# daysun/grid_ndt

Measured on AMD Instinct MI355X. Metric: NDT grid-build throughput (bin + mean/cov + eigen + labels + ordering), higher is better.
Workload: dtype f64

## Files before the change

grid_ndt_amd/_lib.py:

```python
import ctypes as C
import os
import subprocess

_CSRC = os.path.join(os.path.dirname(os.path.abspath(__file__)), "csrc")
_ROOT = os.path.dirname(os.path.dirname(os.path.abspath(__file__)))
LIB_PATH = os.path.join(_CSRC, "libgndt.so")
SOURCES = ["gndt_api_core.hip", "gndt_api_table.hip", "gndt_api_build.hip", "gndt_api_dist.hip", "gndt_api_cost.hip", "gndt_api_query.hip",
           "gndt_api_crop.hip", "gndt_api_raster.hip", "gndt_api_clear.hip", "gndt_api_io.hip", "gndt_codec.cpp", "gndt_io.cpp"]
HEADERS = ["gndt_handle.hpp", "gndt_kernels.hpp", "gndt_table.hpp", "gndt_cost.hpp", "gndt_query.hpp", "gndt_ray.hpp", "gndt_crop.hpp", "gndt_pack.hpp", "gndt_partition.hpp", "gndt_bucket3.hpp", "gndt_blocked.hpp", "gndt_tile.hpp", "gndt_exchange.hpp", "gndt_math.hpp", os.path.join(_ROOT, "include", "gndt.h")]

GNDT_OK = 0
ERR_NAMES = {0: "OK", 1: "INVALID", 2: "NO_DEVICE", 3: "HIP", 4: "KEY_RANGE", 5: "CAPACITY", 6: "NOMEM", 7: "PEER"}


class GndtError(RuntimeError):
    def __init__(self, code, msg):
        super().__init__(f"gndt error {code} ({ERR_NAMES.get(code, '?')}): {msg}")
        self.code = code


class Params(C.Structure):
    _fields_ = [("grid_len", C.c_float), ("z_len", C.c_float), ("slope_interval", C.c_float),
                ("demand", C.c_int32), ("min_points", C.c_int32), ("device_id", C.c_int32),
                ("strategy", C.c_int32), ("max_points_hint", C.c_uint64), ("max_nodes_hint", C.c_uint64)]
# ... 146 lines not shown
    L.gndt_build.argtypes = [H, vp, sz, sz]
    L.gndt_build_device.argtypes = [H, vp, sz, sz, vp]
    L.gndt_update.argtypes = [H, vp, sz, sz]
    L.gndt_update_device.argtypes = [H, vp, sz, sz, vp]
    L.gndt_remove.argtypes = [H, vp, sz, sz]
    L.gndt_remove_device.argtypes = [H, vp, sz, sz, vp]
    L.gndt_reset.argtypes = [H, vp]
    L.gndt_accumulate_device.argtypes = [H, vp, sz, sz, u64, vp]
    L.gndt_finalize_device.argtypes = [H, vp]
    L.gndt_sync.argtypes = [H, C.POINTER(u64), C.POINTER(u64), C.POINTER(u64)]
    L.gndt_export_device.argtypes = [H, C.POINTER(Cells)]
    L.gndt_export.argtypes = [H, C.POINTER(Cells)]
    L.gndt_export_host.argtypes = [H, C.POINTER(Cells)]
    L.gndt_reserve.argtypes = [H, u64, u64]
    L.gndt_set_deferred_emit.argtypes = [H, C.c_int]
    L.gndt_set_deferred_emit.restype = C.c_int
    L.gndt_reserve.restype = C.c_int
    L.gndt_export_host.restype = C.c_int
    L.gndt_stats_export_device.argtypes = [H, C.POINTER(Stats), vp]
    L.gndt_stats_merge_device.argtypes = [H, C.POINTER(Stats), vp]
    L.gndt_shard_stats_device.argtypes = [H, vp, C.c_size_t, C.c_size_t, u64, C.POINTER(Stats), vp]
    L.gndt_finalize_stats_device.argtypes = [H, C.POINTER(Stats), u64, vp]
    L.gndt_get_origin.argtypes = [H, C.POINTER(C.c_float)]
    L.gndt_pcd_read.argtypes = [C.c_char_p, C.POINTER(Pcd), C.c_char_p]
    L.gndt_pcd_free.argtypes = [C.POINTER(Pcd)]
    L.gndt_pcd_free.restype = None
    L.gndt_pack_points_device.argtypes = [H, vp, C.c_size_t, C.POINTER(PointLayout), vp, C.POINTER(u64), vp]
    L.gndt_build_cloud.argtypes = [H, vp, C.c_size_t, C.POINTER(PointLayout)]
    L.gndt_compute_cost.argtypes = [H, C.POINTER(C.c_float), C.POINTER(Robot), vp]
    L.gndt_cost_export_device.argtypes = [H, C.POINTER(vp), C.POINTER(vp), C.POINTER(CostStats)]
    L.gndt_cost_export.argtypes = [H, vp, vp, C.POINTER(CostStats)]
    L.gndt_query_device.argtypes = [H, vp, sz, sz, C.c_int32, vp, vp, vp, vp]
    L.gndt_query.argtypes = [H, vp, sz, sz, C.c_int32, vp, vp, vp]
    L.gndt_crop_device.argtypes = [H, C.POINTER(CropBox), C.c_int32, vp]
    L.gndt_crop.argtypes = [H, C.POINTER(CropBox), C.c_int32]
    L.gndt_crop_box_from_world.argtypes = [C.POINTER(C.c_float), C.c_float, C.POINTER(C.c_float), C.POINTER(C.c_float), C.POINTER(CropBox)]
    L.gndt_raster_shape.argtypes = [C.POINTER(CropBox), C.POINTER(C.c_uint32), C.POINTER(C.c_uint32)]
    L.gndt_raster_device.argtypes = [H, C.POINTER(CropBox), C.c_int32, C.c_float, C.POINTER(RasterLayers), vp]
    L.gndt_raster.argtypes = [H, C.POINTER(CropBox), C.c_int32, C.c_float, C.POINTER(RasterLayers)]
    L.gndt_clear_rays_device.argtypes = [H, C.POINTER(C.c_float), vp, sz, sz, C.POINTER(ClearParams), vp, C.POINTER(ClearStats), vp]
    L.gndt_clear_rays.argtypes = [H, C.POINTER(C.c_float), vp, sz, sz, C.POINTER(ClearParams), vp, C.POINTER(ClearStats)]
    L.gndt_trans_morton_xyz.argtypes = [C.POINTER(C.c_float), C.c_float, C.c_float, C.POINTER(C.c_float), C.c_char_p,
                                        C.POINTER(C.c_int32), C.POINTER(C.c_int32), C.POINTER(C.c_int32), C.c_char_p]
    L.gndt_count_morton.argtypes = [C.c_int32, C.c_int32, C.c_char_p]
    L.gndt_morton_to_xy.argtypes = [C.c_int32, C.POINTER(C.c_int32), C.POINTER(C.c_int32)]
    L.gndt_pack_key.argtypes = [C.c_int32, C.c_int32, C.c_int32]
    L.gndt_pack_key.restype = u64
    L.gndt_unpack_key.argtypes = [u64, C.POINTER(C.c_int32), C.POINTER(C.c_int32), C.POINTER(C.c_int32)]
    L.gndt_unpack_key.restype = None
    L.gndt_set_profiling.argtypes = [H, C.c_int]
    L.gndt_get_phase_times.argtypes = [H, C.POINTER(C.c_double)]
    L.gndt_debug_bucket_phases.argtypes = [H, C.POINTER(C.c_double), C.POINTER(C.c_uint32)]
    L.gndt_debug_bucket_phases.restype = C.c_int
    L.gndt_debug_retry_count.argtypes = [H, C.POINTER(u64)]
    L.gndt_debug_retry_count.restype = C.c_int
    L.gndt_debug_enable_stamps.argtypes = [C.c_int]
    L.gndt_debug_enable_stamps.restype = C.c_int
    L.gndt_warmup.argtypes = [C.c_void_p, C.c_uint64]
    L.gndt_warmup.restype = C.c_int
    L.gndt_debug_set_option.argtypes = [C.c_int, C.c_double]
    L.gndt_debug_set_option.restype = C.c_int
    L.gndt_debug_set_fp_bits.argtypes = [C.c_int]
    L.gndt_debug_set_fp_bits.restype = C.c_int
    L.gndt_debug_fp_clashes.argtypes = [H, C.POINTER(u64)]
    L.gndt_debug_fp_clashes.restype = C.c_int
    L.gndt_debug_second_pass_buckets.argtypes = [H, C.POINTER(u64)]
    L.gndt_debug_second_pass_buckets.restype = C.c_int
    L.gndt_debug_fail_next_alloc.argtypes = [H, C.c_int]
    L.gndt_debug_fail_next_alloc.restype = C.c_int
    L.gndt_comm_unique_id.argtypes = [C.c_char_p]
    L.gndt_comm_create.argtypes = [C.c_char_p, C.c_int32, C.c_int32, C.c_int32, C.POINTER(vp)]
    L.gndt_comm_destroy.argtypes = [vp]
    L.gndt_comm_create_threads.argtypes = [C.c_int32, C.c_int32, C.POINTER(vp)]
    L.gndt_comm_create_threads.restype = C.c_int
    L.gndt_comm_destroy.restype = None
    L.gndt_comm_last_error.restype = C.c_char_p
    L.gndt_comm_selftest.argtypes = [H, vp, C.POINTER(CommSelftest), vp]
    L.gndt_comm_selftest.restype = C.c_int
    L.gndt_build_global_device.argtypes = [H, vp, vp, C.c_size_t, C.c_size_t, u64, u64, C.POINTER(ExchangeTimes), vp]
    L.gndt_owner_of_columns.argtypes = [vp, vp, C.c_size_t, C.c_uint32, vp]
    L.gndt_owner_of_columns.restype = C.c_int
    L.gndt_owner_sample_device.argtypes = [H, vp, C.c_size_t, C.c_size_t, C.POINTER(vp), C.POINTER(u64), vp]
    L.gndt_owner_map_device.argtypes = [H, vp, C.c_uint32, vp]
    L.gndt_owner_sample_device.restype = L.gndt_owner_map_device.restype = C.c_int
    L.gndt_owner_split_device.argtypes = [H, vp, C.c_size_t, C.c_size_t, u64, u64, C.c_uint32, C.POINTER(vp), C.POINTER(u64), C.POINTER(u64), vp]
    L.gndt_build_records_device.argtypes = [H, vp, C.c_size_t, u64, vp]
    L.gndt_build_records2_device.argtypes = [H, vp, C.c_size_t, vp, C.c_size_t, u64, vp]
    L.gndt_build_records2_device.restype = C.c_int
    L.gndt_owned_columns_device.argtypes = [H, C.POINTER(vp), C.POINTER(u64), vp]
    L.gndt_owned_global_rows_device.argtypes = [H, vp, u64, u64, C.POINTER(vp), C.POINTER(u64), C.POINTER(u64), vp]
    L.gndt_build_owned_device.argtypes = [H, vp, vp, C.c_size_t, C.c_size_t, u64, u64, C.POINTER(vp), C.POINTER(OwnedInfo), vp]
    L.gndt_gather_owned_map_device.argtypes = [H, vp, C.c_int32, vp]
    L.gndt_owned_pack_rows_device.argtypes = [H, C.POINTER(vp), C.POINTER(u64), vp]
    L.gndt_adopt_rows_device.argtypes = [H, vp, u64, u64, u64, u64, vp]
    for name in ("gndt_gather_owned_map_device", "gndt_owned_pack_rows_device", "gndt_adopt_rows_device"):
        getattr(L, name).restype = C.c_int
    for name in ("gndt_comm_unique_id", "gndt_comm_create", "gndt_build_global_device", "gndt_owner_split_device",
                 "gndt_build_records_device", "gndt_owned_columns_device", "gndt_owned_global_rows_device", "gndt_build_owned_device"):
        getattr(L, name).restype = C.c_int
    L.gndt_locality_sample.argtypes = [H, vp, C.c_size_t, C.c_size_t, C.c_uint32, C.POINTER(C.c_double), vp]
    L.gndt_locality_sample.restype = C.c_int
    L.gndt_last_strategy.argtypes = [H]
    L.gndt_last_strategy.restype = C.c_int
    L.gndt_device_info.argtypes = [C.c_int32, C.c_char_p, C.POINTER(C.c_int32), C.POINTER(u64)]
    for name in ("gndt_create", "gndt_set_origin", "gndt_build", "gndt_build_device", "gndt_update", "gndt_update_device",
                 "gndt_remove", "gndt_remove_device",
# ... 11 lines not shown
```

grid_ndt_amd/csrc/gndt_api_build.hip:

```cpp
#include <atomic>

#include "gndt_handle.hpp"
#include "gndt_bucket3.hpp"
#include "gndt_blocked.hpp"
using namespace gndt;
using namespace gndt_host;

namespace gndt_host {

int launch_order_and_emit(gndt_handle* h, uint64_t words, int m0, hipStream_t s, bool grouped, bool counters_to_host, bool tab_end, uint32_t advance,
                          bool partial) {
    auto& q = h->part;
    const bool dest_scans = grouped && !partial && !tab_end && words <= kDestScanMax && tuning().dest_scans;
    if (dest_scans) {
    } else if (words <= kScanSmallMax) {
        hipLaunchKernelGGL(k_scan_small, dim3(1), dim3(1024), 0, s, (const uint32_t*)q.word_weight, (uint32_t)words, q.word_base);
    } else {
        const uint32_t nbw = (uint32_t)((words + kScanChunk - 1) / kScanChunk);
        hipLaunchKernelGGL(k_scan_reduce<false>, dim3(nbw), dim3(kScanThreads), 0, s, q.word_weight, (const uint32_t*)nullptr,
                           (uint32_t)words, q.bsum_words);
        hipLaunchKernelGGL(k_scan_apply<false>, dim3(nbw), dim3(kScanThreads), 0, s, q.word_weight, (const uint32_t*)nullptr,
                           (uint32_t)words, q.bsum_words, q.word_base);
    }
    HIP_TRY(h, hipGetLastError());
// ... 478 lines not shown
    h->results_valid = false;
    h->map_in_table = false;
    h->stream_pos = index_range ? index_range : n;
    h->last_stream = s;
    return GNDT_OK;
}

int partition_recheck_after_replay(gndt_handle* h) {
    auto& P = h->pending;
    auto& q = h->part;
    if (P.active || !P.done_serial || P.done_serial != h->result_serial || P.stats_only || P.records || h->map_in_table || !q.h_pc ||
        (!h->results_valid && !P.replay_failed))
        return GNDT_OK;
    if (!(q.h_pc->part_overflow | q.h_pc->lds_overflow | q.h_pc->stage_overflow)) {
        if (P.replay_failed) { P.replay_failed = false; h->results_valid = true; }
        return GNDT_OK;
    }
    h->results_valid = false;
    P.replay_failed = true;
    h->err = "a build replayed from a hipGraph ran out of room (LDS tables " + std::to_string(q.h_pc->lds_overflow) + ", partition regions " +
             std::to_string(q.h_pc->part_overflow) + ", staging rows " + std::to_string(q.h_pc->stage_overflow) +
             "): the capture is sized for the cloud it was recorded on — build this cloud eagerly (gndt_build_device + gndt_sync), then capture again";
    return GNDT_ERR_CAPACITY;
}

static void blocked_decide(gndt_handle* h, const gndt_handle::Pending& P) {
    auto& q = h->part;
    const uint64_t n = P.n + P.n2;
    if (!tuning().blocked || P.stats_only || P.records || P.captured || !P.two_level || P.blocked || h->ever_captured) return;
    if (h->P.strategy != GNDT_STRATEGY_AUTO && h->P.strategy != GNDT_STRATEGY_PARTITION && h->P.strategy != GNDT_STRATEGY_PARTITION_TWO_LEVEL) return;
    if (q.blk_state != 0 && n <= q.blk_n + q.blk_n / 4 && n + n / 4 >= q.blk_n) return;
    q.blk_state = -1; q.blk_n = n;
    if (!(q.pair_ratio >= 0.0 && q.pair_ratio <= 0.02)) return;
    const uint64_t nodes = h->h_cnt->num_nodes;
    if (nodes < 1024 || nodes > h->out_cap) return;
    hipStream_t s = P.s;
    if (!q.d_extent) {
        if (hipMalloc(&q.d_extent, 8 * sizeof(uint32_t)) != hipSuccess) { (void)hipGetLastError(); return; }
        if (hipHostMalloc(&q.h_extent, 8 * sizeof(uint32_t)) != hipSuccess) { (void)hipGetLastError(); return; }
    }
    for (int k = 0; k < 8; ++k) q.h_extent[k] = k < 3 ? 0xFFFFFFFFu : 0u;
    if (hipMemcpyAsync(q.d_extent, q.h_extent, 8 * sizeof(uint32_t), hipMemcpyHostToDevice, s) != hipSuccess) { (void)hipGetLastError(); return; }
    hipLaunchKernelGGL(k_key_extent, dim3(64), dim3(1024), 0, s, (const int32_t*)h->out.sx, (const int32_t*)h->out.sy, (const int32_t*)h->out.sz,
                       (const uint32_t*)h->out.count, (uint32_t)nodes, q.d_extent);
    if (hipMemcpyAsync(q.h_extent, q.d_extent, 8 * sizeof(uint32_t), hipMemcpyDeviceToHost, s) != hipSuccess || hipStreamSynchronize(s) != hipSuccess) {
        (void)hipGetLastError();
        return;
    }
    const int64_t bias = 1ll << 30;
    const int64_t x0 = (int64_t)q.h_extent[0] - bias, y0 = (int64_t)q.h_extent[1] - bias, z0 = (int64_t)q.h_extent[2] - bias;
    const int64_t X = (int64_t)q.h_extent[3] - bias - x0 + 1, Y = (int64_t)q.h_extent[4] - bias - y0 + 1, Z = (int64_t)q.h_extent[5] - bias - z0 + 1;
    const uint64_t biggest = q.h_extent[6];
    if (X <= 0 || Y <= 0 || Z <= 0 || Z > 32) return;
    int shz = 0;
    while ((1 << shz) < Z) ++shz;
    for (; shz <= 5; ++shz) {
        const int shx = (9 - shz + 1) / 2, shy = 9 - shz - shx;
        const uint64_t nx = (uint64_t)((X + (1ll << shx) - 1) >> shx), ny = (uint64_t)((Y + (1ll << shy) - 1) >> shy);
        const uint64_t B = nx * ny;
        if (B < 64 || B > (uint64_t)kMaxFan * kMaxFan) continue;
        const uint64_t per_block = n / B;
        if (per_block > 5000) continue;
        if (per_block < 1500) break;
        if (biggest * 4 > per_block) break;
        if (nodes * 8 < B * 512) break;
        const int64_t zpad = ((1ll << shz) - Z) / 2;
        q.blk_map = BlockMap{1, (int)(x0 - (1ll << shx)), (int)(y0 - (1ll << shy)), (int)(z0 - zpad), shx, shy, shz, (int)nx + 2, (int)ny + 2};
        q.blk_buckets = (uint32_t)((nx + 2) * (ny + 2));
        if (q.blk_buckets > (uint64_t)kMaxFan * kMaxFan) { q.blk_map.on = 0; continue; }
        q.blk_state = 1;
        if (tuning().verbose)
            fprintf(stderr, "[gndt] blocked buckets for clouds of ~%llu points: box %lld x %lld x %lld, blocks of %d x %d columns x %d levels, %llu buckets of ~%llu points\n",
                    (unsigned long long)n, (long long)X, (long long)Y, (long long)Z, 1 << shx, 1 << shy, 1 << shz, (unsigned long long)B, (unsigned long long)per_block);
        return;
    }
}

int partition_resolve(gndt_handle* h) {
    auto& P = h->pending;
    if (!P.active) return GNDT_OK;
    auto& q = h->part;
    const int env_slots = tuning().bucket_slots;
    int rc = GNDT_OK;
    for (;;) {
        if (hipStreamSynchronize(P.s) != hipSuccess) { P.active = false; h->err = "hipStreamSynchronize failed"; return GNDT_ERR_HIP; }
        bool again = false;
        if (P.two_level && P.mean1 > 0) {
            q.fill1_ratio = q.h_pc->max_fill1 / P.mean1;
            if (tuning().verbose)
                fprintf(stderr, "[gndt] two-level partition: fullest level-1 region %.2fx the mean, overflow %u\n",
                        q.h_pc->max_fill1 / P.mean1, q.h_pc->part_overflow);
        }
        if (tuning().verbose && (q.h_pc->part_overflow | q.h_pc->lds_overflow | q.h_pc->stage_overflow))
            fprintf(stderr, "[gndt] build of %zu points, attempt %d (%d-slot tables, %llu nodes expected): region overflow %u, table overflow %u, "
                            "staging overflow %u -> re-run\n", P.n, P.attempt, P.bslots, (unsigned long long)P.nodes_est, q.h_pc->part_overflow,
                    q.h_pc->lds_overflow, q.h_pc->stage_overflow);
        if (P.blocked && (q.h_pc->blk_miss | q.h_pc->part_overflow)) {
            q.blk_state = -1;
            P.no_block = true;
            --P.attempt;
            again = true;
        } else if (q.h_pc->part_overflow) {
            if (P.one_level) q.one_level_ok = false;
            else ++q.two_level_failures;
            --P.attempt;
            again = true;
        } else if (q.h_pc->lds_overflow) {
            const bool without_retry = P.bslots == 512 && !P.retry_pass && tuning().retry_pass != 0 && !env_slots;
            q.retry_pass = true;
            const uint64_t b1024 = buckets_for(P.n + P.n2, P.nodes_est, 1024, P.load_pct ? P.load_pct : q.load_pct);
            if (without_retry) {
                --P.attempt;
            } else if (P.bslots == 512 && !env_slots && P.n + P.n2 <= (1u << 20) && b1024 < 384 && (P.load_pct ? P.load_pct : q.load_pct) > 35) {
                P.load_pct = 35;
                --P.attempt;
            } else if (P.attempt >= 1 || env_slots) {
                const bool few = q.h_pc->lds_overflow * 64u <= q.last_buckets;
                P.nodes_est = few ? P.nodes_est + (P.nodes_est * 2) / 5 : P.nodes_est * 2;
            }
            again = true;
        } else if (q.h_pc->stage_overflow) {
            const uint64_t true_nodes = h->h_cnt->num_nodes;
            const uint64_t want = true_nodes + true_nodes / 8 + 1024;
            if (want > P.stage_want) --P.attempt;
            P.stage_want = want;
            P.rows_floor = want;
// ... 141 lines not shown
        HIP_TRY(h, hipMalloc(&q.bucket_base, ((size_t)Bexact + 1) * 4));
        q.bucket_cap = (uint32_t)Bexact;
    }
    if ((rc = reserve_table(h, std::max<uint64_t>(max_nodes, std::max<uint64_t>(1024, n / 4)), h->own_stream))) return rc;
    HIP_TRY(h, hipStreamSynchronize(h->own_stream));
    if ((rc = ensure_stage(h, std::max<uint64_t>(1024, h->cap / 2 + 1)))) return rc;
    if ((rc = ensure_raw(h, q.stage_cap))) return rc;
    if ((rc = ensure_out(h, q.stage_cap))) return rc;
    return GNDT_OK;
}

int gndt_debug_retry_count(gndt_handle* h, uint64_t* retries) {
    if (!h || !retries) return GNDT_ERR_INVALID;
    *retries = h->part.retries_total;
    return GNDT_OK;
}

int gndt_debug_second_pass_buckets(gndt_handle* h, uint64_t* buckets) {
    if (!h || !buckets) return GNDT_ERR_INVALID;
    *buckets = h->part.retry_seen;
    return GNDT_OK;
}

int gndt_debug_enable_stamps(int on) { tuning_force_stamps(on != 0); return GNDT_OK; }
int gndt_debug_set_option(int option, double value) { return tuning_set_option(option, value); }

int gndt_debug_set_fp_bits(int bits) { tuning_force_fp_bits(bits); return GNDT_OK; }

int gndt_debug_fp_clashes(gndt_handle* h, uint64_t* buckets) {
    if (!h || !buckets) return GNDT_ERR_INVALID;
    *buckets = h->part.h_pc ? h->part.h_pc->fp_clashes : 0;
    return GNDT_OK;
}

int gndt_debug_bucket_phases(gndt_handle* h, double cycles_out[10], uint32_t* buckets_out) {
    if (!h || !cycles_out) return GNDT_ERR_INVALID;
    auto& q = h->part;
    if (!q.dbg || !q.last_buckets) { h->err = "no stamps: call gndt_debug_enable_stamps(1) before a PARTITION build"; return GNDT_ERR_INVALID; }
    HIP_TRY(h, hipSetDevice(h->device));
    HIP_TRY(h, hipStreamSynchronize(h->last_stream));
    std::vector<unsigned long long> t((size_t)q.last_buckets * 16);
    HIP_TRY(h, hipMemcpy(t.data(), q.dbg, t.size() * sizeof(unsigned long long), hipMemcpyDeviceToHost));
    for (int k = 0; k < 10; ++k) cycles_out[k] = 0.0;
    for (uint32_t b = 0; b < q.last_buckets; ++b) {
        const unsigned long long* s = &t[(size_t)b * 16];
        for (int k = 0; k < 6; ++k) if (s[k + 1] > s[k]) cycles_out[k] += (double)(s[k + 1] - s[k]);
        for (int k = 0; k < 4; ++k) cycles_out[6 + k] += (double)s[8 + k];
    }
    for (int k = 0; k < 10; ++k) cycles_out[k] /= q.last_buckets;
    if (buckets_out) *buckets_out = q.last_buckets;
    return GNDT_OK;
}

}

namespace {
__global__ void k_warm_fill(float* __restrict__ xyz, uint32_t n, uint32_t stride_floats, float gl, float zl) {
    for (uint32_t i = blockIdx.x * blockDim.x + threadIdx.x; i < n; i += gridDim.x * blockDim.x) {
        uint32_t a = i * 0x9E3779B1u + 0x7F4A7C15u; a ^= a >> 15; a *= 0x85EBCA77u; a ^= a >> 13;
        uint32_t b = a * 0xC2B2AE3Du + 0x165667B1u; b ^= b >> 16;
        uint32_t c = b * 0x27D4EB2Fu + 0x9E3779B1u; c ^= c >> 15;
        float* p = xyz + (size_t)i * stride_floats;
        p[0] = ((float)(a >> 8) * (1.0f / 16777216.0f) - 0.5f) * 100.0f * gl;
        p[1] = ((float)(b >> 8) * (1.0f / 16777216.0f) - 0.5f) * 100.0f * gl;
        p[2] = ((float)(c >> 8) * (1.0f / 16777216.0f) - 0.5f) * 4.0f * zl;
        if (stride_floats == 4) p[3] = 0.f;
    }
}
std::atomic<uint64_t> g_warm_points[64];
}

int gndt_warmup(gndt_handle* h, uint64_t expected_points) {
    if (!h) return GNDT_ERR_INVALID;
    HIP_TRY(h, hipSetDevice(h->device));
    {
        hipStreamCaptureStatus cap = hipStreamCaptureStatusNone;
        (void)hipStreamIsCapturing(h->own_stream, &cap);
        if (cap != hipStreamCaptureStatusNone) { h->err = "gndt_warmup: not under stream capture"; return GNDT_ERR_INVALID; }
    }
    uint64_t n = expected_points ? expected_points : (h->P.max_points_hint ? h->P.max_points_hint : 200000);
    const uint64_t reserve_points = expected_points ? expected_points : h->P.max_points_hint;
    n = std::min<uint64_t>(std::max<uint64_t>(n, 1u << 16), 4u << 20);
    const bool known_device = h->device >= 0 && h->device < 64;
    int rc = GNDT_OK;
    const uint64_t seen = known_device ? g_warm_points[h->device].load(std::memory_order_acquire) : 0;
    const bool loaded = seen && n <= seen + seen / 4 && n + n / 4 >= seen;
    if (!loaded) {
        hipStream_t s = h->own_stream;
        float* cloud = nullptr;
        HIP_TRY(h, hipMalloc(&cloud, (size_t)n * 16));
        auto run = [&](int strategy, uint32_t stride_floats, bool update, bool flood) -> int {
            gndt_params tp = h->P;
            tp.strategy = strategy; tp.max_points_hint = 0; tp.max_nodes_hint = 0;
            gndt_handle* t = nullptr;
            int r = create_handle(&tp, &t, s);
            if (r) { h->err = std::string("gndt_warmup: ") + gndt_last_error(nullptr); return r; }
            const float origin[3] = {0.f, 0.f, 0.f};
            hipLaunchKernelGGL(k_warm_fill, dim3(512), dim3(256), 0, s, cloud, (uint32_t)n, stride_floats, tp.grid_len, tp.z_len);
            r = gndt_set_origin(t, origin);
            for (int k = 0; k < 2 && !r; ++k) {
                r = gndt_build_device(t, cloud, (size_t)n, stride_floats * 4u, nullptr);
                if (!r) r = gndt_sync(t, nullptr, nullptr, nullptr);
            }
            if (!r && update) {
                r = gndt_update_device(t, cloud, (size_t)std::min<uint64_t>(n, 1u << 17), stride_floats * 4u, nullptr);
                if (!r) r = gndt_sync(t, nullptr, nullptr, nullptr);
// ... 26 lines not shown
```

grid_ndt_amd/csrc/gndt_blocked.hpp:

```cpp
#pragma once
#include <hip/hip_runtime.h>
#include <stdint.h>

#include "gndt_bucket3.hpp"

namespace gndt {

constexpr uint32_t kBlkChunk = 2048;
constexpr int kBlkPer = (int)kBlkChunk / 512;
constexpr uint32_t kBlkNone = 0xFFFFFFFFu;
struct BlockedLds {
    float4 image[kBlkChunk];
    uint32_t hist[2][512];
    uint32_t wpre[2][8];
    uint2 fz[512];
    uint32_t cpre[512];
    uint32_t wave_tot[8];
    uint32_t n_nodes, n_cols, n_slopes, stage_base, err_range, miss;
};

template <int T>
__global__ void __launch_bounds__(T) __attribute__((amdgpu_waves_per_eu(6, 6))) k_bucket_blocked(const float4* __restrict__ recs, BucketRanges ranges, uint32_t num_buckets, GridParams P,
                                                      RawNode* __restrict__ stage, uint32_t stage_cap,
                                                      uint32_t* __restrict__ ord_cf, uint32_t* __restrict__ ord_idx, ColumnOrder O,
                                                      Counters* __restrict__ cnt, PartCounters* __restrict__ pc,
                                                      unsigned long long* __restrict__ dbg) {
    static_assert(T == 512, "one table slot per thread");
    __shared__ BlockedLds L;
    const int tid = threadIdx.x;
    const BlockMap K = P.blk;
    const int sh_xy = K.shx + K.shy;
    const uint32_t col_mask = (1u << sh_xy) - 1u, n_levels = 1u << K.shz;
    if (blockIdx.x == 0 && tid == 0) { const uint32_t e = pc->l1_err; if (e) atomicAdd(&cnt->err_key_range, e); }
    for (uint32_t bucket = blockIdx.x; bucket < num_buckets; bucket += gridDim.x) {
#define GNDT_STAMPB(k) do { if (dbg && tid == 0) dbg[(size_t)bucket * 16 + (k)] = __builtin_amdgcn_s_memtime(); } while (0)
        uint32_t lo, hi;
        bucket_range(ranges, bucket, lo, hi);
        GNDT_STAMPB(0);
        const int bx0 = K.x0 + (int)((bucket / (uint32_t)K.ny) << K.shx), by0 = K.y0 + (int)((bucket % (uint32_t)K.ny) << K.shy);
        uint32_t s = (uint32_t)tid;
        asm volatile("" : "+v"(s));
        const uint32_t zero = s - (uint32_t)tid;
        float f_len = P.grid_len, f_zlen = P.z_len, f_ox = P.ox, f_oy = P.oy, f_oz = P.oz;
        asm volatile("" : "+s"(f_len), "+s"(f_zlen), "+s"(f_ox), "+s"(f_oy), "+s"(f_oz));
        const double hx = 0.5 * (double)f_len, hz = 0.5 * (double)f_zlen;
        const double ox = (double)f_ox, oy = (double)f_oy, oz = (double)f_oz;
        L.hist[0][s] = zero; L.hist[1][s] = zero;
        if (s < 16) L.wpre[s >> 3][s & 7] = zero;
        if (s == 0) { L.n_nodes = zero; L.n_cols = zero; L.n_slopes = zero; L.stage_base = zero; L.err_range = zero; L.miss = zero; }
        lds_barrier();
        GNDT_STAMPB(1);
        const uint32_t col = s & col_mask, lz = s >> sh_xy;
        const int cxi = bx0 + (int)(col & ((1u << K.shx) - 1u)), cyi = by0 + (int)(col >> K.shx), czi = K.z0 + (int)lz;
        const int nsx = cxi >= 0 ? cxi + 1 : cxi, nsy = cyi >= 0 ? cyi + 1 : cyi, nsz = czi >= 0 ? czi + 1 : czi;
        const double ctx = fma((double)(float)(nsx > 0 ? 2 * nsx - 1 : 2 * nsx + 1), hx, ox),
                     cty = fma((double)(float)(nsy > 0 ? 2 * nsy - 1 : 2 * nsy + 1), hx, oy),
                     ctz = fma((double)(float)(nsz > 0 ? 2 * nsz - 1 : 2 * nsz + 1), hz, oz);
        const uint32_t n_rec = hi - lo, n_chunks = (n_rec + kBlkChunk - 1u) / kBlkChunk;
        uint32_t my_n = 0, my_first = 0xFFFFFFFFu;
        double sums[9];
#pragma unroll
        for (int j = 0; j < 9; ++j) sums[j] = 0.0;
        float4 rec[kBlkPer];
#pragma unroll
        for (int j = 0; j < kBlkPer; ++j) rec[j] = make_float4(0.f, 0.f, 0.f, 0.f);
        if (lo < hi) {
#pragma unroll
            for (int j = 0; j < kBlkPer; ++j) rec[j] = recs[min(lo + (uint32_t)(j * T + tid), hi - 1u)];
        }
        for (uint32_t ch = 0; ch < n_chunks; ++ch) {
            const uint32_t par = ch & 1u, c0 = lo + ch * kBlkChunk;
            uint32_t slot_rank[kBlkPer];
#pragma unroll
            for (int j = 0; j < kBlkPer; ++j) {
                bool use = c0 + (uint32_t)(j * T + tid) < hi;
                bool und = false;
                float fx = axis_ceil_try(rec[j].x, P.ox, P.inv_grid, und);
                float fy = axis_ceil_try(rec[j].y, P.oy, P.inv_grid, und);
                float fz = axis_ceil_try(rec[j].z, P.oz, P.inv_z, und);
                if (und) {
                    fx = ceilf(fabsf(rec[j].x - P.ox) / P.grid_len);
                    fy = ceilf(fabsf(rec[j].y - P.oy) / P.grid_len);
                    fz = ceilf(fabsf(rec[j].z - P.oz) / P.z_len);
                }
                bool ok = true;
                int sx, sy, sz;
                double v0, v1, v2;
                axis_index_offset(rec[j].x, P.ox, fx, (float)kMaxXY, hx, ox, ok, sx, v0);
                axis_index_offset(rec[j].y, P.oy, fy, (float)kMaxXY, hx, oy, ok, sy, v1);
                axis_index_offset(rec[j].z, P.oz, fz, (float)kMaxZ, hz, oz, ok, sz, v2);
                (void)v0; (void)v1; (void)v2;
                if (use && !ok) { atomicAdd(&L.err_range, 1u); use = false; }
                const uint32_t lx = (uint32_t)(contiguous_index(sx) - bx0), ly = (uint32_t)(contiguous_index(sy) - by0),
                               lz2 = (uint32_t)(contiguous_index(sz) - K.z0);
                if (use && ((lx >> K.shx) | (ly >> K.shy) | (lz2 >> K.shz)) != 0u) { L.miss = 1u; use = false; }
                const uint32_t rs = (lz2 << sh_xy) | (ly << K.shx) | lx;
                slot_rank[j] = use ? (rs << 16) | atomicAdd(&L.hist[par][rs], 1u) : kBlkNone;
            }
            lds_barrier();
            {
                const uint32_t c = L.hist[par][s];
                uint32_t incl = c;
                const int lane = tid & 63, wv = tid >> 6;
                for (int off = 1; off < 64; off <<= 1) { const uint32_t t = (uint32_t)__shfl_up((int)incl, off, 64); if (lane >= off) incl += t; }
                const uint32_t wtot = (uint32_t)__shfl((int)incl, 63, 64);
                L.hist[par][s] = incl - c;
                if (lane > wv && lane < T / 64 && wtot) atomicAdd(&L.wpre[par][lane], wtot);
                L.hist[par ^ 1u][s] = 0u;
                if (tid < T / 64) L.wpre[par ^ 1u][tid] = 0u;
                lds_barrier();
#pragma unroll
                for (int j = 0; j < kBlkPer; ++j) {
                    const uint32_t sr = slot_rank[j];
                    if (sr != kBlkNone) L.image[L.hist[par][sr >> 16] + L.wpre[par][sr >> 22] + (sr & 0xFFFFu)] = rec[j];
                }
                const uint32_t b0 = incl - c + L.wpre[par][wv];
                if (ch + 1u < n_chunks) {
#pragma unroll
                    for (int j = 0; j < kBlkPer; ++j) rec[j] = recs[min(c0 + kBlkChunk + (uint32_t)(j * T + tid), hi - 1u)];
                }
                lds_barrier();
#pragma unroll 1
                for (uint32_t i = b0; i < b0 + c; ++i) {
                    const float4 r = L.image[i];
                    const double v0 = (double)r.x - ctx, v1 = (double)r.y - cty, v2 = (double)r.z - ctz;
                    const uint32_t iw = __float_as_uint(r.w);
                    uint32_t cn = 1u, cf = iw;
                    double w0 = v0, w1 = v1, w2 = v2;
                    if (__any((iw & kWeight64Flag) != 0u)) {
                        cn = record_weight(iw); cf = record_index(iw);
                        const double wf = (double)cn;
                        w0 = wf * v0; w1 = wf * v1; w2 = wf * v2;
                    }
                    my_n += cn; my_first = min(my_first, cf);
                    sums[0] += w0; sums[1] += w1; sums[2] += w2;
                    sums[3] += w0 * v0; sums[4] += w0 * v1; sums[5] += w0 * v2;
                    sums[6] += w1 * v1; sums[7] += w1 * v2; sums[8] += w2 * v2;
                }
            }
        }
        const bool live = my_n != 0u;
        {
            const uint32_t w = (uint32_t)__popcll(__ballot(live));
            if ((tid & 63) == 0 && w) atomicAdd(&L.n_nodes, w);
        }
        lds_barrier();
        GNDT_STAMPB(2);
        if (L.miss) {
            if (tid == 0) atomicAdd(&pc->blk_miss, 1u);
            lds_barrier();
            continue;
        }
        const uint32_t M = L.n_nodes;
        uint32_t stage_base_reg = 0;
        if (tid == T - 1 && M) stage_base_reg = atomicAdd(&cnt->num_nodes, M);
        if (tid == 0 && L.err_range) atomicAdd(&cnt->err_key_range, L.err_range);
        const float cz = (live && my_n >= (uint32_t)P.min_points) ? node_mean_z(my_n, sums[2], axis_centre(nsz, P.oz, P.z_len)) : 0.f;
        L.fz[s] = make_uint2(my_first, __float_as_uint(cz));
        lds_barrier();
        uint32_t icol = 0, ncol = 0, cfirst = 0xFFFFFFFFu;
        bool up = false, down = false;
        if (live || s <= col_mask) {
            for (uint32_t k0 = 0; k0 < n_levels; k0 += 4) {
                uint2 tt[4];
#pragma unroll
                for (int j = 0; j < 4; ++j) tt[j] = L.fz[min(((k0 + (uint32_t)j) << sh_xy) | col, 511u)];
#pragma unroll
                for (int j = 0; j < 4; ++j) {
                    const uint32_t k = k0 + (uint32_t)j, tf = tt[j].x;
                    if (k >= n_levels || tf == 0xFFFFFFFFu) continue;
                    ++ncol;
                    cfirst = min(cfirst, tf);
                    if (k == lz) continue;
                    icol += (tf < my_first) ? 1u : 0u;
                    if (k == lz + 1u || k + 1u == lz) {
                        const float oz2 = (tf < my_first) ? __uint_as_float(tt[j].y) : 0.f;
                        const bool far = fabsf(oz2 - cz) > P.slope_interval;
                        if (k == lz + 1u) up = far; else down = far;
                    }
                }
            }
        }
        {
            const uint32_t my_col_nodes = s <= col_mask ? ncol : 0u;
            uint32_t incl = my_col_nodes;
            const int lane = tid & 63;
            for (int off = 1; off < 64; off <<= 1) { const uint32_t t = (uint32_t)__shfl_up((int)incl, off, 64); if (lane >= off) incl += t; }
            if (s <= col_mask) L.cpre[s] = incl - my_col_nodes;
            if (lane == 63) L.wave_tot[tid >> 6] = incl;
            if (s <= col_mask && my_col_nodes) atomicAdd(&L.n_cols, 1u);
            if (tid == T - 1) L.stage_base = stage_base_reg;
            lds_barrier();
        }
        GNDT_STAMPB(3);
        const uint32_t sbase = L.stage_base;
        if (sbase + M > stage_cap) {
            if (tid == 0 && M) atomicAdd(&pc->stage_overflow, M);
            lds_barrier();
            continue;
        }
        uint32_t my_slopes = 0;
        if (live) {
            uint32_t fl = (my_n >= (uint32_t)P.min_points) ? 1u : 0u;
            if (fl) {
                bool slope = true;
                if (P.demand == 0) slope = !up; else down = false;
                if (slope) { fl |= 2u; if (down) fl |= 4u; ++my_slopes; }
            }
            RawNode row;
            row.key = pack_key(nsx, nsy, nsz); row.count = my_n; row.first = my_first;
#pragma unroll
            for (int j = 0; j < 9; ++j) row.sum[j] = sums[j];
            row.info = fl | (icol << 3);
            row.ncol = ncol;
            uint32_t cbase = L.cpre[col];
            for (uint32_t w = 0; w < (col >> 6); ++w) cbase += L.wave_tot[w];
            const uint32_t dst = sbase + cbase + icol;
            stage[dst] = row;
            ord_cf[dst] = cfirst;
            ord_idx[dst] = icol ? icol : (kOrdHeadFlag | ncol);
            if (icol == 0) note_column(O, cfirst, ncol);
        }
        if (my_slopes) atomicAdd(&L.n_slopes, my_slopes);
        lds_barrier();
        if (tid == 0) {
            if (L.n_cols | L.n_slopes) atomicAdd(&pc->cols_slopes, ((unsigned long long)L.n_slopes << 32) | (unsigned long long)L.n_cols);
        }
        GNDT_STAMPB(4);
        lds_barrier();
#undef GNDT_STAMPB
    }
}

static __global__ void __launch_bounds__(1024) k_key_extent(const int32_t* __restrict__ sx, const int32_t* __restrict__ sy, const int32_t* __restrict__ sz,
                                                            const uint32_t* __restrict__ count, uint32_t n, uint32_t* __restrict__ out) {
    __shared__ uint32_t red[7];
    if (threadIdx.x < 3) red[threadIdx.x] = 0xFFFFFFFFu;
    else if (threadIdx.x < 7) red[threadIdx.x] = 0u;
    __syncthreads();
    uint32_t mn[3] = {0xFFFFFFFFu, 0xFFFFFFFFu, 0xFFFFFFFFu}, mx[3] = {0u, 0u, 0u}, big = 0u;
    for (uint32_t i = blockIdx.x * blockDim.x + threadIdx.x; i < n; i += gridDim.x * blockDim.x) {
        const uint32_t c[3] = {(uint32_t)(contiguous_index(sx[i]) + (1 << 30)), (uint32_t)(contiguous_index(sy[i]) + (1 << 30)),
                               (uint32_t)(contiguous_index(sz[i]) + (1 << 30))};
#pragma unroll
        for (int k = 0; k < 3; ++k) { mn[k] = min(mn[k], c[k]); mx[k] = max(mx[k], c[k]); }
        big = max(big, count[i]);
    }
#pragma unroll
    for (int k = 0; k < 3; ++k) {
        for (int off = 32; off > 0; off >>= 1) {
            mn[k] = min(mn[k], (uint32_t)__shfl_down((int)mn[k], off, 64));
            mx[k] = max(mx[k], (uint32_t)__shfl_down((int)mx[k], off, 64));
        }
    }
    for (int off = 32; off > 0; off >>= 1) big = max(big, (uint32_t)__shfl_down((int)big, off, 64));
    if ((threadIdx.x & 63) == 0) {
#pragma unroll
        for (int k = 0; k < 3; ++k) { atomicMin(&red[k], mn[k]); atomicMax(&red[3 + k], mx[k]); }
        atomicMax(&red[6], big);
    }
    __syncthreads();
    if (threadIdx.x < 3) atomicMin(&out[threadIdx.x], red[threadIdx.x]);
    else if (threadIdx.x < 7) atomicMax(&out[threadIdx.x], red[threadIdx.x]);
}

}
```

grid_ndt_amd/csrc/gndt_kernels.hpp:

```cpp
#pragma once
#include <hip/hip_runtime.h>
#include <stdint.h>

#include "gndt_math.hpp"

namespace gndt {

struct NodeAcc {
    double s[9];
    uint32_t count;
    uint32_t first;
};
static_assert(sizeof(NodeAcc) == 80, "NodeAcc layout");

struct SlotAux {
    float mean_z;
    uint32_t flags;
};

struct Counters {
    uint32_t num_nodes;
    uint32_t num_columns;
    uint32_t num_slopes;
    uint32_t err_key_range;
    uint32_t err_table_full;
    uint32_t stream_pos;
    uint32_t prev_nodes;
    uint32_t epoch;
    uint32_t n_touched;
    uint32_t n_tcols;
    uint32_t n_work;
    uint32_t n_dead;
    uint32_t err_remove;
    uint32_t first_word;
    uint32_t ticket;
    uint32_t table_gen;
    uint32_t table_unclean;
    uint32_t part_owned;
};

struct BlockMap {
    int on;
    int x0, y0, z0;
    int shx, shy, shz;
    int nx, ny;
};
struct GridParams {
    float ox, oy, oz;
    float grid_len, z_len, slope_interval;
    int demand, min_points;
    float inv_grid, inv_z;
    BlockMap blk;
};

struct OutView {
    int32_t *sx, *sy, *sz;
    uint32_t *count, *first_idx;
    float *mean, *cov, *rough, *normal;
    uint32_t* flags;
};

constexpr int kBlock = 256;

__device__ __forceinline__ uint32_t find_or_insert(uint64_t* __restrict__ keys, uint32_t cap_mask, uint64_t key,
                                                   bool& inserted) {
    inserted = false;
    uint32_t slot = (uint32_t)mix64(key) & cap_mask;
    for (uint32_t probe = 0; probe <= cap_mask; ++probe) {
        uint64_t k = keys[slot];
        if (k == key) return slot;
        if (k == kEmptyKey) {
            unsigned long long old = atomicCAS((unsigned long long*)&keys[slot], (unsigned long long)kEmptyKey,
                                               (unsigned long long)key);
            if (old == kEmptyKey) { inserted = true; return slot; }
            if (old == key) return slot;
        }
        slot = (slot + 1) & cap_mask;
    }
    return cap_mask + 1;
}

__device__ __forceinline__ void append_new_nodes(bool inserted, uint32_t slot, uint32_t* __restrict__ node_slot,
                                                 uint32_t* __restrict__ index_of_slot, Counters* __restrict__ cnt) {
    const unsigned long long m = __ballot(inserted);
    if (m == 0ull) return;
    const int lane = threadIdx.x & 63;
    const int leader = (int)__builtin_ctzll(m);
    uint32_t base = 0;
    if (lane == leader) base = atomicAdd(&cnt->num_nodes, (uint32_t)__popcll(m));
    base = (uint32_t)__shfl((int)base, leader, 64);
    if (inserted) {
        const uint32_t idx = base + (uint32_t)__popcll(m & ((1ull << lane) - 1ull));
        node_slot[idx] = slot;
        index_of_slot[slot] = idx;
    }
}

// ... 351 lines not shown
```

grid_ndt_amd/map2d.py:

```python
import ctypes as C
import os

import numpy as np

from . import _lib
from ._lib import Cells, ClearParams, ClearStats, CropBox, CostStats, ExchangeTimes, GndtError, OwnedInfo, Params, Pcd, PointLayout, RasterLayers, Robot, Stats

DEMANDS = {"slope": 0, "true": 1}
FLAG_HAS_STATS, FLAG_SLOPE, FLAG_DOWN = 1, 2, 4


_HIP_STREAM_LEGACY = 1


def _stream_ptr(stream):
    if stream is None:
        try:
            import torch
            if torch.cuda.is_available():
                return C.c_void_p(torch.cuda.current_stream().cuda_stream or _HIP_STREAM_LEGACY)
        except ImportError:
            pass
        return C.c_void_p(0)
    if hasattr(stream, "cuda_stream"):
# ... 372 lines not shown
        return r.value

    def last_strategy(self):
        return int(self._L.gndt_last_strategy(self._h))

    def phase_times_ms(self):
        arr = (C.c_double * 10)()
        self._check(self._L.gndt_get_phase_times(self._h, arr))
        names = self.PHASES[self.last_strategy()]
        return {k: arr[i] for i, k in enumerate(names)}

    def retry_count(self):
        r = C.c_uint64()
        self._check(self._L.gndt_debug_retry_count(self._h, C.byref(r)))
        return int(r.value)

    def enable_stamps(self, on=True):
        self._L.gndt_debug_enable_stamps(int(bool(on)))

    def reserve(self, max_points, max_nodes=0, demand="slope"):
        self._ensure(demand, need_origin=False)
        self._check(self._L.gndt_reserve(self._h, int(max_points), int(max_nodes)))

    def warmup(self, expected_points=0, demand="slope"):
        self._ensure(demand, need_origin=False)
        self._check(self._L.gndt_warmup(self._h, int(expected_points)))

    def set_deferred_emit(self, on=True, demand="slope"):
        self._ensure(demand)
        self._check(self._L.gndt_set_deferred_emit(self._h, int(bool(on))))

    DEBUG_VERBOSE, DEBUG_TILE_RATIO, DEBUG_COST_ONE_WORKGROUP, DEBUG_QUERY_ILP = 1, 2, 3, 4

    @staticmethod
    def set_debug_option(option, value):
        rc = _lib.lib().gndt_debug_set_option(int(option), float(value))
        if rc:
            raise _lib.GndtError(rc, f"gndt_debug_set_option({option}, {value})")

    def set_fp_bits(self, bits):
        self._L.gndt_debug_set_fp_bits(int(bits))

    def fp_clashes(self):
        r = C.c_uint64()
        self._check(self._L.gndt_debug_fp_clashes(self._h, C.byref(r)))
        return int(r.value)

    def debug_bucket_phases(self):
        arr = (C.c_double * 10)()
        nb = C.c_uint32()
        self._check(self._L.gndt_debug_bucket_phases(self._h, arr, C.byref(nb)))
        names = ("clear", "accumulate", "columns", "rows", "-", "-", "acc:0", "acc:1", "acc:2", "acc:3")
        return dict(zip(names, list(arr))), nb.value

    def computeCost(self, goal, robot=None, stream=None):
        g = (C.c_float * 3)(*[float(v) for v in goal])
        rb = None
        if robot is not None:
            d = dict(radius=0.25, reachable_height=0.15, max_rough=100.0, max_angle_deg=30.0)
            d.update(robot)
            rb = C.byref(Robot(d["radius"], d["reachable_height"], d["max_rough"], d["max_angle_deg"]))
        self._check(self._L.gndt_compute_cost(self._h, g, rb, _stream_ptr(stream)))
        st = CostStats()
        self._check(self._L.gndt_cost_export(self._h, None, None, C.byref(st)))
        return self._cost_stats(st)

    @staticmethod
    def _cost_stats(st):
        return {"rc": int(st.goal_status), "ring": int(st.ring), "levels": int(st.levels), "traversable": int(st.traversable),
                "closed": int(st.closed), "check_pushes": int(st.check_pushes), "ring_store": int(st.ring_store)}

    def cost_export(self):
        n, _, _ = self.sync()
        h = np.zeros(n, np.float32)
        state = np.zeros(n, np.uint32)
        st = CostStats()
        self._check(self._L.gndt_cost_export(self._h, h.ctypes.data, state.ctypes.data, C.byref(st)))
        out = self._cost_stats(st)
        out.update(h=h, state=state.astype(np.uint8))
        return out

    QUERY_MODES = {"node": 0, "nearest_slope": 1}
    NO_ROW = -1

    def query(self, points, mode="node", cost=False, stream=None):
        if self._h is None:
            self._ensure(self._demand if self._demand is not None else "slope", need_origin=False)
        m = self.QUERY_MODES[mode] if isinstance(mode, str) else int(mode)
        ptr, n, stride, on_dev, keep = self._as_input(points)
        if on_dev:
            import torch
            rows = torch.empty(n, dtype=torch.int32, device=keep.device)
            h = torch.empty(n, dtype=torch.float32, device=keep.device) if cost else None
            state = torch.empty(n, dtype=torch.int32, device=keep.device) if cost else None
            p = lambda t: C.c_void_p(t.data_ptr() if t is not None and n else 0)
            self._check(self._L.gndt_query_device(self._h, C.c_void_p(ptr if n else 0), n, stride, m, p(rows), p(h), p(state),
                                                  _stream_ptr(stream)))
        else:
            rows = np.empty(n, np.int32)
            h = np.empty(n, np.float32) if cost else None
            state = np.empty(n, np.int32) if cost else None
            p = lambda a: C.c_void_p(a.ctypes.data if a is not None and n else 0)
            self._check(self._L.gndt_query(self._h, C.c_void_p(ptr if n else 0), n, stride, m, p(rows), p(h), p(state)))
        return (rows, h, state) if cost else rows

    CROP_MODES = {"keep_inside": 0, "drop_inside": 1}
# ... 212 lines not shown
```

include/gndt.h:

```cpp
#ifndef GNDT_H
#define GNDT_H

#include <stddef.h>
#include <stdint.h>

#ifdef __cplusplus
extern "C" {
#endif

typedef struct gndt_handle gndt_handle;

enum {
    GNDT_OK = 0,
    GNDT_ERR_INVALID = 1,
    GNDT_ERR_NO_DEVICE = 2,
    GNDT_ERR_HIP = 3,
    GNDT_ERR_KEY_RANGE = 4,
    GNDT_ERR_CAPACITY = 5,
    GNDT_ERR_NOMEM = 6,
    GNDT_ERR_PEER = 7
};

enum { GNDT_DEMAND_SLOPE = 0, GNDT_DEMAND_TRUE = 1 };

// ... 182 lines not shown
int gndt_raster_shape(const gndt_crop_box* box, uint32_t* width, uint32_t* height);
int gndt_raster_device(gndt_handle* h, const gndt_crop_box* box, int32_t mode, float z_ref, const gndt_raster_layers* out_dev,
                       void* hip_stream);
int gndt_raster(gndt_handle* h, const gndt_crop_box* box, int32_t mode, float z_ref, const gndt_raster_layers* out_host);

enum { GNDT_CLEAR_COUNT_ONLY = 1 };
#define GNDT_CLEAR_PROTECTED 0x80000000u
typedef struct gndt_clear_params {
    float max_range;
    float end_margin;
    uint32_t min_passes;
    uint32_t flags;
} gndt_clear_params;
typedef struct gndt_clear_stats {
    uint64_t rays, skipped, protected_rows, cleared;
} gndt_clear_stats;
int gndt_clear_rays_device(gndt_handle* h, const float origin_xyz[3], const void* xyz_dev, size_t n, size_t stride_bytes,
                           const gndt_clear_params* p, uint32_t* passes_out_dev, gndt_clear_stats* stats, void* hip_stream);
int gndt_clear_rays(gndt_handle* h, const float origin_xyz[3], const void* xyz_host, size_t n, size_t stride_bytes,
                    const gndt_clear_params* p, uint32_t* passes_out_host, gndt_clear_stats* stats);

typedef struct gndt_point_layout {
    uint32_t point_step, offset_x, offset_y, offset_z;
} gndt_point_layout;

typedef struct gndt_pcd {
    uint64_t num_points;
    gndt_point_layout layout;
    int32_t data_kind;
    int32_t reserved;
    void* data;
} gndt_pcd;
int gndt_pcd_read(const char* path, gndt_pcd* out, char err[256]);
void gndt_pcd_free(gndt_pcd* pcd);

int gndt_pack_points_device(gndt_handle* h, const void* raw_dev, size_t n, const gndt_point_layout* layout,
                            float* xyz_out_dev, uint64_t* n_valid, void* hip_stream);
int gndt_build_cloud(gndt_handle* h, const void* raw_host, size_t n, const gndt_point_layout* layout);

int gndt_trans_morton_xyz(const float origin[3], float grid_len, float z_len, const float p[3],
                          char* quadrant, int32_t* nx, int32_t* ny, int32_t* sz, char key_out[16]);
int gndt_count_morton(int32_t a, int32_t b, char out[16]);
int gndt_morton_to_xy(int32_t morton, int32_t* a, int32_t* b);
uint64_t gndt_pack_key(int32_t sx, int32_t sy, int32_t sz);
void gndt_unpack_key(uint64_t key, int32_t* sx, int32_t* sy, int32_t* sz);

#define GNDT_NUM_PHASES 10
int gndt_set_profiling(gndt_handle* h, int enable);
int gndt_get_phase_times(gndt_handle* h, double ms_out[GNDT_NUM_PHASES]);
int gndt_locality_sample(gndt_handle* h, const void* xyz_dev, size_t n, size_t stride_bytes, uint32_t tiles, double* points_per_partial,
                         void* hip_stream);
int gndt_last_strategy(const gndt_handle* h);
int gndt_debug_bucket_phases(gndt_handle* h, double cycles_out[10], uint32_t* buckets_out);
int gndt_debug_retry_count(gndt_handle* h, uint64_t* retries);
int gndt_debug_enable_stamps(int on);
#define GNDT_DEBUG_VERBOSE 1
#define GNDT_DEBUG_TILE_RATIO 2
#define GNDT_DEBUG_COST_ONE_WORKGROUP 3
#define GNDT_DEBUG_QUERY_ILP 4
#define GNDT_DEBUG_CLEAR_EXTENT 5
int gndt_debug_set_option(int option, double value);
int gndt_debug_set_fp_bits(int bits);
int gndt_debug_fp_clashes(gndt_handle* h, uint64_t* buckets);
int gndt_debug_second_pass_buckets(gndt_handle* h, uint64_t* buckets);
int gndt_debug_fail_next_alloc(gndt_handle* h, int site);

int gndt_device_info(int32_t device_id, char name_out[128], int32_t* compute_units, uint64_t* hbm_bytes);

#ifdef __cplusplus
}
#endif
#endif
```

Baseline: 35660.

## Size blocked buckets to the cloud's exact z-extent and skip empty buckets

```diff
diff --git a/grid_ndt_amd/_lib.py b/grid_ndt_amd/_lib.py
--- a/grid_ndt_amd/_lib.py
+++ b/grid_ndt_amd/_lib.py
@@ -222,6 +222,8 @@
     L.gndt_get_phase_times.argtypes = [H, C.POINTER(C.c_double)]
     L.gndt_debug_bucket_phases.argtypes = [H, C.POINTER(C.c_double), C.POINTER(C.c_uint32)]
     L.gndt_debug_bucket_phases.restype = C.c_int
+    L.gndt_debug_bucket_stamps.argtypes = [H, C.POINTER(C.c_ulonglong), u64, C.POINTER(C.c_uint32)]
+    L.gndt_debug_bucket_stamps.restype = C.c_int
     L.gndt_debug_retry_count.argtypes = [H, C.POINTER(u64)]
     L.gndt_debug_retry_count.restype = C.c_int
     L.gndt_debug_enable_stamps.argtypes = [C.c_int]
diff --git a/grid_ndt_amd/csrc/gndt_api_build.hip b/grid_ndt_amd/csrc/gndt_api_build.hip
--- a/grid_ndt_amd/csrc/gndt_api_build.hip
+++ b/grid_ndt_amd/csrc/gndt_api_build.hip
@@ -554,26 +554,26 @@
     const int64_t X = (int64_t)q.h_extent[3] - bias - x0 + 1, Y = (int64_t)q.h_extent[4] - bias - y0 + 1, Z = (int64_t)q.h_extent[5] - bias - z0 + 1;
     const uint64_t biggest = q.h_extent[6];
     if (X <= 0 || Y <= 0 || Z <= 0 || Z > 32) return;
-    int shz = 0;
-    while ((1 << shz) < Z) ++shz;
-    for (; shz <= 5; ++shz) {
-        const int shx = (9 - shz + 1) / 2, shy = 9 - shz - shx;
+    int sh_xy = 0;
+    while ((Z << (sh_xy + 1)) <= 512) ++sh_xy;
+    for (; sh_xy >= 0; --sh_xy) {
+        const int shx = (sh_xy + 1) / 2, shy = sh_xy - shx;
         const uint64_t nx = (uint64_t)((X + (1ll << shx) - 1) >> shx), ny = (uint64_t)((Y + (1ll << shy) - 1) >> shy);
         const uint64_t B = nx * ny;
-        if (B < 64 || B > (uint64_t)kMaxFan * kMaxFan) continue;
+        if (B > (uint64_t)kMaxFan * kMaxFan) break;
+        if (B < 64) continue;
         const uint64_t per_block = n / B;
         if (per_block > 5000) continue;
         if (per_block < 1500) break;
         if (biggest * 4 > per_block) break;
-        if (nodes * 8 < B * 512) break;
-        const int64_t zpad = ((1ll << shz) - Z) / 2;
-        q.blk_map = BlockMap{1, (int)(x0 - (1ll << shx)), (int)(y0 - (1ll << shy)), (int)(z0 - zpad), shx, shy, shz, (int)nx + 2, (int)ny + 2};
+        if (nodes * 8 < B * ((uint64_t)Z << sh_xy)) break;
+        q.blk_map = BlockMap{1, (int)(x0 - (1ll << shx)), (int)(y0 - (1ll << shy)), (int)z0, shx, shy, (int)Z, (int)nx + 2, (int)ny + 2};
         q.blk_buckets = (uint32_t)((nx + 2) * (ny + 2));
-        if (q.blk_buckets > (uint64_t)kMaxFan * kMaxFan) { q.blk_map.on = 0; continue; }
+        if (q.blk_buckets > (uint64_t)kMaxFan * kMaxFan) { q.blk_map.on = 0; break; }
         q.blk_state = 1;
         if (tuning().verbose)
-            fprintf(stderr, "[gndt] blocked buckets for clouds of ~%llu points: box %lld x %lld x %lld, blocks of %d x %d columns x %d levels, %llu buckets of ~%llu points\n",
-                    (unsigned long long)n, (long long)X, (long long)Y, (long long)Z, 1 << shx, 1 << shy, 1 << shz, (unsigned long long)B, (unsigned long long)per_block);
+            fprintf(stderr, "[gndt] blocked buckets for clouds of ~%llu points: box %lld x %lld x %lld, blocks of %d x %d columns x %lld levels, %llu buckets of ~%llu points\n",
+                    (unsigned long long)n, (long long)X, (long long)Y, (long long)Z, 1 << shx, 1 << shy, (long long)Z, (unsigned long long)B, (unsigned long long)per_block);
         return;
     }
 }
@@ -821,6 +821,18 @@
     return GNDT_OK;
 }
 
+int gndt_debug_bucket_stamps(gndt_handle* h, unsigned long long* out, uint64_t cap, uint32_t* buckets_out) {
+    if (!h || (!out && cap)) return GNDT_ERR_INVALID;
+    auto& q = h->part;
+    if (!q.dbg || !q.last_buckets) { h->err = "no stamps: call gndt_debug_enable_stamps(1) before a PARTITION build"; return GNDT_ERR_INVALID; }
+    HIP_TRY(h, hipSetDevice(h->device));
+    HIP_TRY(h, hipStreamSynchronize(h->last_stream));
+    const uint64_t n = std::min<uint64_t>(cap, (uint64_t)q.last_buckets * 16);
+    if (n) HIP_TRY(h, hipMemcpy(out, q.dbg, n * sizeof(unsigned long long), hipMemcpyDeviceToHost));
+    if (buckets_out) *buckets_out = q.last_buckets;
+    return GNDT_OK;
+}
+
 }
 
 namespace {
diff --git a/grid_ndt_amd/csrc/gndt_blocked.hpp b/grid_ndt_amd/csrc/gndt_blocked.hpp
--- a/grid_ndt_amd/csrc/gndt_blocked.hpp
+++ b/grid_ndt_amd/csrc/gndt_blocked.hpp
@@ -17,6 +17,8 @@
     uint32_t cpre[512];
     uint32_t wave_tot[8];
     uint32_t n_nodes, n_cols, n_slopes, stage_base, err_range, miss;
+    unsigned long long lap_t;
+    uint32_t lap[5], runs[4];
 };
 
 template <int T>
@@ -30,12 +32,14 @@
     const int tid = threadIdx.x;
     const BlockMap K = P.blk;
     const int sh_xy = K.shx + K.shy;
-    const uint32_t col_mask = (1u << sh_xy) - 1u, n_levels = 1u << K.shz;
+    const uint32_t col_mask = (1u << sh_xy) - 1u, n_levels = (uint32_t)K.nz;
     if (blockIdx.x == 0 && tid == 0) { const uint32_t e = pc->l1_err; if (e) atomicAdd(&cnt->err_key_range, e); }
     for (uint32_t bucket = blockIdx.x; bucket < num_buckets; bucket += gridDim.x) {
 #define GNDT_STAMPB(k) do { if (dbg && tid == 0) dbg[(size_t)bucket * 16 + (k)] = __builtin_amdgcn_s_memtime(); } while (0)
+#define GNDT_LAP(k) do { if (dbg && tid == 0) { const unsigned long long t_ = __builtin_amdgcn_s_memtime(); L.lap[k] += (uint32_t)(t_ - L.lap_t); L.lap_t = t_; } } while (0)
         uint32_t lo, hi;
         bucket_range(ranges, bucket, lo, hi);
+        if (lo == hi) continue;
         GNDT_STAMPB(0);
         const int bx0 = K.x0 + (int)((bucket / (uint32_t)K.ny) << K.shx), by0 = K.y0 + (int)((bucket % (uint32_t)K.ny) << K.shy);
         uint32_t s = (uint32_t)tid;
@@ -48,8 +52,10 @@
         L.hist[0][s] = zero; L.hist[1][s] = zero;
         if (s < 16) L.wpre[s >> 3][s & 7] = zero;
         if (s == 0) { L.n_nodes = zero; L.n_cols = zero; L.n_slopes = zero; L.stage_base = zero; L.err_range = zero; L.miss = zero; }
+        if (dbg && s < 9) { if (s < 5) L.lap[s] = 0u; else L.runs[s - 5] = 0u; }
         lds_barrier();
         GNDT_STAMPB(1);
+        if (dbg && tid == 0) L.lap_t = __builtin_amdgcn_s_memtime();
         const uint32_t col = s & col_mask, lz = s >> sh_xy;
         const int cxi = bx0 + (int)(col & ((1u << K.shx) - 1u)), cyi = by0 + (int)(col >> K.shx), czi = K.z0 + (int)lz;
         const int nsx = cxi >= 0 ? cxi + 1 : cxi, nsy = cyi >= 0 ? cyi + 1 : cyi, nsz = czi >= 0 ? czi + 1 : czi;
@@ -70,6 +76,11 @@
         }
         for (uint32_t ch = 0; ch < n_chunks; ++ch) {
             const uint32_t par = ch & 1u, c0 = lo + ch * kBlkChunk;
+            if (dbg) {
+#pragma unroll
+                for (int j = 0; j < kBlkPer; ++j) asm volatile("" :: "v"(rec[j].x), "v"(rec[j].y), "v"(rec[j].z), "v"(rec[j].w));
+                GNDT_LAP(0);
+            }
             uint32_t slot_rank[kBlkPer];
 #pragma unroll
             for (int j = 0; j < kBlkPer; ++j) {
@@ -93,11 +104,18 @@
                 if (use && !ok) { atomicAdd(&L.err_range, 1u); use = false; }
                 const uint32_t lx = (uint32_t)(contiguous_index(sx) - bx0), ly = (uint32_t)(contiguous_index(sy) - by0),
                                lz2 = (uint32_t)(contiguous_index(sz) - K.z0);
-                if (use && ((lx >> K.shx) | (ly >> K.shy) | (lz2 >> K.shz)) != 0u) { L.miss = 1u; use = false; }
-                const uint32_t rs = (lz2 << sh_xy) | (ly << K.shx) | lx;
-                slot_rank[j] = use ? (rs << 16) | atomicAdd(&L.hist[par][rs], 1u) : kBlkNone;
+                if (use && (((lx >> K.shx) | (ly >> K.shy)) != 0u || lz2 >= n_levels)) { L.miss = 1u; use = false; }
+                slot_rank[j] = use ? (lz2 << sh_xy) | (ly << K.shx) | lx : kBlkNone;
+            }
+#pragma unroll
+            for (int j = 0; j < kBlkPer; ++j) {
+                const bool use = slot_rank[j] != kBlkNone;
+                const uint32_t rs = use ? slot_rank[j] : s;
+                const uint32_t rk = atomicAdd(&L.hist[par][rs], use ? 1u : 0u);
+                slot_rank[j] = use ? (rs << 16) | rk : kBlkNone;
             }
             lds_barrier();
+            GNDT_LAP(1);
             {
                 const uint32_t c = L.hist[par][s];
                 uint32_t incl = c;
@@ -109,17 +127,30 @@
                 L.hist[par ^ 1u][s] = 0u;
                 if (tid < T / 64) L.wpre[par ^ 1u][tid] = 0u;
                 lds_barrier();
+                GNDT_LAP(2);
+                if (dbg && ch == 0u) {
+                    uint32_t rmax = c;
+                    for (int off = 32; off > 0; off >>= 1) rmax = max(rmax, (uint32_t)__shfl_xor((int)rmax, off, 64));
+                    const uint32_t nlive = (uint32_t)__popcll(__ballot(c != 0u));
+                    if (c) atomicAdd(&L.runs[1], c);
+                    if (lane == 0 && nlive) { atomicAdd(&L.runs[0], rmax); atomicAdd(&L.runs[2], nlive); atomicAdd(&L.runs[3], 1u); }
+                }
+                uint32_t dst[kBlkPer];
 #pragma unroll
                 for (int j = 0; j < kBlkPer; ++j) {
-                    const uint32_t sr = slot_rank[j];
-                    if (sr != kBlkNone) L.image[L.hist[par][sr >> 16] + L.wpre[par][sr >> 22] + (sr & 0xFFFFu)] = rec[j];
-                }
+                    const uint32_t sl = (slot_rank[j] >> 16) & 511u;
+                    dst[j] = L.hist[par][sl] + L.wpre[par][sl >> 6] + (slot_rank[j] & 0xFFFFu);
+                }
+#pragma unroll
+                for (int j = 0; j < kBlkPer; ++j)
+                    if (slot_rank[j] != kBlkNone) L.image[dst[j]] = rec[j];
                 const uint32_t b0 = incl - c + L.wpre[par][wv];
                 if (ch + 1u < n_chunks) {
 #pragma unroll
                     for (int j = 0; j < kBlkPer; ++j) rec[j] = recs[min(c0 + kBlkChunk + (uint32_t)(j * T + tid), hi - 1u)];
                 }
                 lds_barrier();
+                GNDT_LAP(3);
 #pragma unroll 1
                 for (uint32_t i = b0; i < b0 + c; ++i) {
                     const float4 r = L.image[i];
@@ -137,6 +168,7 @@
                     sums[3] += w0 * v0; sums[4] += w0 * v1; sums[5] += w0 * v2;
                     sums[6] += w1 * v1; sums[7] += w1 * v2; sums[8] += w2 * v2;
                 }
+                if (dbg) { lds_barrier(); GNDT_LAP(4); }
             }
         }
         const bool live = my_n != 0u;
@@ -146,6 +178,16 @@
         }
         lds_barrier();
         GNDT_STAMPB(2);
+        if (dbg && tid == 0) {
+            dbg[(size_t)bucket * 16 + 8] = L.lap[0];
+            dbg[(size_t)bucket * 16 + 9] = L.lap[1];
+            dbg[(size_t)bucket * 16 + 10] = L.lap[2] + L.lap[3];
+            dbg[(size_t)bucket * 16 + 11] = L.lap[4];
+            dbg[(size_t)bucket * 16 + 12] = L.lap[3];
+            dbg[(size_t)bucket * 16 + 13] = L.runs[0];
+            dbg[(size_t)bucket * 16 + 14] = L.runs[1];
+            dbg[(size_t)bucket * 16 + 15] = ((unsigned long long)L.runs[2] << 32) | L.runs[3];
+        }
         if (L.miss) {
             if (tid == 0) atomicAdd(&pc->blk_miss, 1u);
             lds_barrier();
@@ -229,6 +271,7 @@
         GNDT_STAMPB(4);
         lds_barrier();
 #undef GNDT_STAMPB
+#undef GNDT_LAP
     }
 }
 
diff --git a/grid_ndt_amd/csrc/gndt_kernels.hpp b/grid_ndt_amd/csrc/gndt_kernels.hpp
--- a/grid_ndt_amd/csrc/gndt_kernels.hpp
+++ b/grid_ndt_amd/csrc/gndt_kernels.hpp
@@ -42,7 +42,8 @@
 struct BlockMap {
     int on;
     int x0, y0, z0;
-    int shx, shy, shz;
+    int shx, shy;
+    int nz;
     int nx, ny;
 };
 struct GridParams {
diff --git a/grid_ndt_amd/map2d.py b/grid_ndt_amd/map2d.py
--- a/grid_ndt_amd/map2d.py
+++ b/grid_ndt_amd/map2d.py
@@ -448,6 +448,13 @@
         self._check(self._L.gndt_debug_bucket_phases(self._h, arr, C.byref(nb)))
         names = ("clear", "accumulate", "columns", "rows", "-", "-", "acc:0", "acc:1", "acc:2", "acc:3")
         return dict(zip(names, list(arr))), nb.value
+
+    def debug_bucket_stamps(self):
+        nb = C.c_uint32()
+        self._check(self._L.gndt_debug_bucket_stamps(self._h, None, 0, C.byref(nb)))
+        out = np.zeros((nb.value, 16), dtype=np.uint64)
+        self._check(self._L.gndt_debug_bucket_stamps(self._h, out.ctypes.data_as(C.POINTER(C.c_ulonglong)), out.size, C.byref(nb)))
+        return out
 
     def computeCost(self, goal, robot=None, stream=None):
         g = (C.c_float * 3)(*[float(v) for v in goal])
diff --git a/include/gndt.h b/include/gndt.h
--- a/include/gndt.h
+++ b/include/gndt.h
@@ -258,6 +258,7 @@
                          void* hip_stream);
 int gndt_last_strategy(const gndt_handle* h);
 int gndt_debug_bucket_phases(gndt_handle* h, double cycles_out[10], uint32_t* buckets_out);
+int gndt_debug_bucket_stamps(gndt_handle* h, unsigned long long* out, uint64_t cap, uint32_t* buckets_out);
 int gndt_debug_retry_count(gndt_handle* h, uint64_t* retries);
 int gndt_debug_enable_stamps(int on);
 #define GNDT_DEBUG_VERBOSE 1
```

Measured after the change: 34700 (median of 2 runs). -2.7%, worse.
